# FitSNAP/FitSNAP

Hardware: AMD Instinct MI355X
Metric: training rows/sec through A^T A + solve, 1000000 x 128 fp64 in total over the GPUs (strong scaling) (higher is better)
Workload: dtype f64

## Files before the change

fitsnap_amd/csrc/fsnap_syrk.hip:

```cpp

#include <utility>

#include "fsnap_device_common.h"
#include "fsnap_kernels.h"

namespace {

__host__ __device__ constexpr int tri_index(int p, int q, int NB) {
    return p * NB - (p * (p - 1)) / 2 + (q - p);
}

__host__ __device__ inline int col_of(int bq, int e, int NB) {
    if ((NB & 1) && bq == NB - 1) return 16 * bq + e;
    return 32 * (bq >> 1) + 2 * e + (bq & 1);
}

__device__ __forceinline__ __amdgpu_buffer_rsrc_t make_rsrc(const void* p, unsigned bytes) {
    return __builtin_amdgcn_make_buffer_rsrc(const_cast<void*>(p), 0, (int)bytes, 0x00020000);
}

__device__ __forceinline__ double xlane_sum_rows(double x) {
    x += __shfl_xor(x, 16, 64);
    x += __shfl_xor(x, 32, 64);
    return x;
}

}

#ifdef FSNAP_TRACE
__device__ unsigned long long fsnap_trace_buf[4096 * 8];
__device__ unsigned long long fsnap_trace_wave[4096 * 16 * 4];
#define FSNAP_TRACE_CLK(v) const unsigned long long v = __builtin_readcyclecounter()
#endif

namespace {

template <int T, int NV>
__device__ __forceinline__ void acc_mfma(double a, double b, d4 (&vt)[NV]) {
    if constexpr (T < 32) {
        asm volatile("v_mfma_f64_16x16x4_f64 a[%2:%3], %0, %1, a[%2:%3]" : : "v"(a), "v"(b), "n"(8 * T), "n"(8 * T + 7));
    } else {
        asm volatile("v_mfma_f64_16x16x4_f64 %0, %1, %2, %0" : "+v"(vt[T - 32]) : "v"(a), "v"(b));
    }
}

template <int R>
__device__ __forceinline__ void acc_zero_reg() {
    asm volatile("v_accvgpr_write_b32 a[%0], 0" : : "n"(R));
}
template <int... R>
__device__ __forceinline__ void acc_zero_all(std::integer_sequence<int, R...>) {
    (acc_zero_reg<R>(), ...);
}

template <int T, int NV>
__device__ __forceinline__ d4 acc_read(const d4 (&vt)[NV]) {
    if constexpr (T >= 32) {
        return vt[T - 32];
    } else {
        unsigned r0, r1, r2, r3, r4, r5, r6, r7;
        asm volatile(
            "v_accvgpr_read_b32 %0, a[%8]\n\tv_accvgpr_read_b32 %1, a[%9]\n\t"
            "v_accvgpr_read_b32 %2, a[%10]\n\tv_accvgpr_read_b32 %3, a[%11]\n\t"
            "v_accvgpr_read_b32 %4, a[%12]\n\tv_accvgpr_read_b32 %5, a[%13]\n\t"
            "v_accvgpr_read_b32 %6, a[%14]\n\tv_accvgpr_read_b32 %7, a[%15]"
            : "=v"(r0), "=v"(r1), "=v"(r2), "=v"(r3), "=v"(r4), "=v"(r5), "=v"(r6), "=v"(r7)
            : "n"(8 * T), "n"(8 * T + 1), "n"(8 * T + 2), "n"(8 * T + 3), "n"(8 * T + 4), "n"(8 * T + 5), "n"(8 * T + 6),
              "n"(8 * T + 7));
        d4 x;
        x[0] = __builtin_bit_cast(double, ((unsigned long long)r1 << 32) | r0);
        x[1] = __builtin_bit_cast(double, ((unsigned long long)r3 << 32) | r2);
        x[2] = __builtin_bit_cast(double, ((unsigned long long)r5 << 32) | r4);
        x[3] = __builtin_bit_cast(double, ((unsigned long long)r7 << 32) | r6);
        return x;
    }
}

template <int TB, int N, int NV, int... U>
__device__ __forceinline__ void acc_read_range(d4 (&tmp)[N], const d4 (&vt)[NV], std::integer_sequence<int, U...>) {
    ((tmp[U] = acc_read<TB + U, NV>(vt)), ...);
}

template <int NB, int P, int NV, int... Q>
__device__ __forceinline__ void acc_row(const double (&V)[NB], d4 (&vt)[NV], std::integer_sequence<int, Q...>) {
    (acc_mfma<tri_index(P, P + Q, NB), NV>(V[P], V[P + Q], vt), ...);
}

template <int NB>
struct RawM {
    u4 pr[NB / 2 > 0 ? NB / 2 : 1];
    u2 tail;
    u4 wp;
};

constexpr unsigned FSNAP_OOB_VOFF = 0xFFFFF000u;

struct WaveBufsP {
    __amdgpu_buffer_rsrc_t A, wp;
    unsigned voffA;
    unsigned voffT;
    unsigned voffP;
    unsigned chunk_bytes;
};

__device__ __forceinline__ u4 load_pack(const WaveBufsP& wb, unsigned cl) {
    return __builtin_amdgcn_raw_buffer_load_b128(wb.wp, wb.voffP, cl * 64u, 0);
}
__device__ __forceinline__ bool pack_keep(const u4& wp) {
    return ((wp[0] | (wp[1] & 0x7FFFFFFFu)) != 0u);
}

template <int NB, bool NT>
__device__ __forceinline__ void issue_rows(RawM<NB>& r, const WaveBufsP& wb, unsigned cl) {
    const unsigned soff = cl * wb.chunk_bytes;
    constexpr int AUX = NT ? 2 : 0;
    const bool keep = pack_keep(r.wp);
    const unsigned va = keep ? wb.voffA : FSNAP_OOB_VOFF;
#pragma unroll
    for (int j = 0; j < NB / 2; ++j) r.pr[j] = __builtin_amdgcn_raw_buffer_load_b128(wb.A, va + 256u * j, soff, AUX);
    if (NB & 1) {
        const unsigned vtl = keep ? wb.voffT : FSNAP_OOB_VOFF;
        r.tail = __builtin_amdgcn_raw_buffer_load_b64(wb.A, vtl, soff, AUX);
    }
}

template <int NB, bool NT>
__device__ __forceinline__ void issue_rows_w(RawM<NB>& r, const u4& wp, const WaveBufsP& wb, unsigned cl) {
    const unsigned soff = cl * wb.chunk_bytes;
    constexpr int AUX = NT ? 2 : 0;
    const bool keep = pack_keep(wp);
    const unsigned va = keep ? wb.voffA : FSNAP_OOB_VOFF;
#pragma unroll
    for (int j = 0; j < NB / 2; ++j) r.pr[j] = __builtin_amdgcn_raw_buffer_load_b128(wb.A, va + 256u * j, soff, AUX);
    if (NB & 1) {
        const unsigned vtl = keep ? wb.voffT : FSNAP_OOB_VOFF;
        r.tail = __builtin_amdgcn_raw_buffer_load_b64(wb.A, vtl, soff, AUX);
    }
}

template <class F, int... I>
__device__ __forceinline__ void wave_p_for_impl(F&& f, std::integer_sequence<int, I...>) {
    (f(std::integral_constant<int, I>{}), ...);
}
template <int N, class F>
__device__ __forceinline__ void wave_p_for(F&& f) {
    wave_p_for_impl(f, std::make_integer_sequence<int, N>{});
}

template <int NB, bool NT, int P>
__device__ __forceinline__ void issue_piece(RawM<NB>& r, const WaveBufsP& wb, unsigned cl, unsigned va, unsigned vtl) {
    constexpr int AUX = NT ? 2 : 0;
    constexpr int NPR = NB / 2;
    const unsigned soff = cl * wb.chunk_bytes;
    if (P < NPR) r.pr[P] = __builtin_amdgcn_raw_buffer_load_b128(wb.A, va + 256u * P, soff, AUX);
    if ((NB & 1) && P == NPR) r.tail = __builtin_amdgcn_raw_buffer_load_b64(wb.A, vtl, soff, AUX);
    static_assert(NPR + (NB & 1) <= NB, "one load piece per MFMA slot");
}

template <int NB, bool FULLK>
__device__ __forceinline__ double weighted_block(const RawM<NB>& r, int j, double wv, int K, int e) {
    if ((NB & 1) && j == NB - 1) {
        const double x = wv * __builtin_bit_cast(double, r.tail);
        if (FULLK) return x;
        return (16 * (NB - 1) + e < K) ? x : 0.0;
    }
    const double x = wv * __builtin_bit_cast(d2, r.pr[j >> 1])[j & 1];
    constexpr int last_pair = (NB & 1) ? -1 : NB / 2 - 1;
    if (FULLK || (j >> 1) != last_pair) return x;
    return (32 * (j >> 1) + 2 * e + (j & 1) < K) ? x : 0.0;
}

template <bool PACK>
__device__ __forceinline__ u4 load_pack_x(const WaveBufsP& wb, const double* lpk, unsigned cl) {
    if constexpr (PACK) return __builtin_bit_cast(u4, *reinterpret_cast<const d2*>(lpk + (size_t)cl * 8));
    else return load_pack(wb, cl);
}

__device__ __forceinline__ void pack_rows_to_lds(const double* __restrict__ b, const double* __restrict__ w,
                                                 const unsigned char* __restrict__ mask, int64_t row0, int64_t nrow,
                                                 unsigned wave_rows, unsigned region_rows, double* lpw, int lane, double* sout) {
    constexpr int PB = 16;
    const __amdgpu_buffer_rsrc_t rb = make_rsrc(b + row0, (unsigned)(nrow * 8));
    const __amdgpu_buffer_rsrc_t rw_ = make_rsrc(w + row0, (unsigned)(nrow * 8));
    const __amdgpu_buffer_rsrc_t rm = make_rsrc(mask + row0, (unsigned)nrow);
    double bb = 0.0, sb = 0.0, cnt = 0.0;
    for (unsigned r0 = 0; r0 < wave_rows; r0 += 64u * PB) {
        u2 bv[PB], wv[PB];
        unsigned char mk[PB];
#pragma unroll
        for (int u = 0; u < PB; ++u) {
            const unsigned row = r0 + 64u * u + (unsigned)lane;
            bv[u] = __builtin_amdgcn_raw_buffer_load_b64(rb, row * 8u, 0, 0);
            wv[u] = __builtin_amdgcn_raw_buffer_load_b64(rw_, row * 8u, 0, 0);
            mk[u] = __builtin_amdgcn_raw_buffer_load_b8(rm, row, 0, 0);
        }
#pragma unroll
        for (int u = 0; u < PB; ++u) {
            const unsigned row = r0 + 64u * u + (unsigned)lane;
            const bool keep = (mk[u] != 0);
            const double wvv = keep ? __builtin_bit_cast(double, wv[u]) : 0.0;
            const double wbv = keep ? wvv * __builtin_bit_cast(double, bv[u]) : 0.0;
            if (row < wave_rows) {
                d2 o;
                o[0] = wvv;
                o[1] = wbv;
                *reinterpret_cast<d2*>(lpw + (size_t)row * 2) = o;
            }
            bb = __builtin_fma(wbv, wbv, bb);
            sb += wbv;
            cnt += keep ? 1.0 : 0.0;
        }
    }
    for (unsigned row = wave_rows + (unsigned)lane; row < region_rows; row += 64u) {
        const d2 z = {0.0, 0.0};
        *reinterpret_cast<d2*>(lpw + (size_t)row * 2) = z;
    }
#pragma unroll
    for (int sh = 1; sh < 64; sh <<= 1) {
        bb += __shfl_xor(bb, sh, 64);
        sb += __shfl_xor(sb, sh, 64);
        cnt += __shfl_xor(cnt, sh, 64);
    }
    if (lane == 0) {
        sout[0] = bb;
        sout[1] = sb;
        sout[2] = cnt;
        sout[3] = 0.0;
    }
}

template <int NB, bool FULLK, bool NT, int P>
__device__ __forceinline__ void acc_slot(double (&V)[NB], const RawM<NB>& RN, double wv, double wbv, double& wbp, int K,
                                         int e, double (&cacc)[NB], RawM<NB>& RF, const WaveBufsP& wb, unsigned cl_fill,
                                         unsigned va, unsigned vtl) {
#if !defined(FSNAP_ACC_ABL) || !(FSNAP_ACC_ABL & 1)
    issue_piece<NB, NT, P>(RF, wb, cl_fill, va, vtl);
#endif
    if (P == 0) cacc[NB - 1] = __builtin_fma(V[NB - 1], wbp, cacc[NB - 1]);
    else cacc[P - 1] = __builtin_fma(V[P - 1], wbv, cacc[P - 1]);
    V[P] = weighted_block<NB, FULLK>(RN, P, wv, K, e);
    if (P == NB - 1) wbp = wbv;
    __builtin_amdgcn_sched_barrier(0);
}

template <int NB, bool FULLK, bool NT, bool PACK, int NV, int... P>
__device__ __forceinline__ void acc_step(double (&V)[NB], d4 (&vt)[NV], RawM<NB>& RF, const RawM<NB>& RN, const WaveBufsP& wb,
                                         const double* lpk, unsigned cl_fill, int K, int e, double (&cacc)[NB], double& wbp,
                                         const u4& PW, const u4& PKEEP, u4& PLOAD, std::integer_sequence<int, P...>) {
    const d2 wpn = __builtin_bit_cast(d2, PW);
    const double wv = wpn[0], wbv = wpn[1];
    const bool keep = pack_keep(PKEEP);
    const unsigned va = keep ? wb.voffA : FSNAP_OOB_VOFF;
    const unsigned vtl = (NB & 1) ? (keep ? wb.voffT : FSNAP_OOB_VOFF) : 0u;
#if !defined(FSNAP_ACC_ABL) || !(FSNAP_ACC_ABL & 1)
    PLOAD = load_pack_x<PACK>(wb, lpk, cl_fill + 2);
#endif
    __builtin_amdgcn_sched_barrier(0);
#if defined(FSNAP_ACC_ABL) && (FSNAP_ACC_ABL & 2)
    (acc_row<NB, P>(V, vt, std::make_integer_sequence<int, NB - P>{}), ...);
    (void)wbv;
#else
    ((acc_row<NB, P>(V, vt, std::make_integer_sequence<int, NB - P>{}),
      acc_slot<NB, FULLK, NT, P>(V, RN, wv, wbv, wbp, K, e, cacc, RF, wb, cl_fill, va, vtl)),
     ...);
#endif
}

constexpr int FSNAP_ACC_LDS_DOUBLES = 20480;
constexpr int FSNAP_ACC_PACK_PAD = 12;

}

template <int NB, bool FULLK, bool NT, bool PACK>
__global__ __launch_bounds__(256) __attribute__((amdgpu_waves_per_eu(1, 1))) void
fsnap_syrk_acc(const double* __restrict__ A, int64_t lda, const double* __restrict__ wpack, int64_t m, int K,
               int64_t chunks_per_wave, double* __restrict__ part, double* __restrict__ cpart,
               const double* __restrict__ bvec, const double* __restrict__ wvec, const unsigned char* __restrict__ mask,
               double* __restrict__ spart) {

    constexpr int NTILE = NB * (NB + 1) / 2;
    constexpr int NV = NTILE > 32 ? NTILE - 32 : 1;
    constexpr int NPART = (NTILE * 1024 + FSNAP_ACC_LDS_DOUBLES - 1) / FSNAP_ACC_LDS_DOUBLES;
    constexpr int PER = (NTILE + NPART - 1) / NPART;
    static_assert(4 * PER * 256 <= FSNAP_ACC_LDS_DOUBLES, "fold part does not fit the LDS");
    __shared__ __attribute__((aligned(16))) double lds[FSNAP_ACC_LDS_DOUBLES];
#ifdef FSNAP_TRACE
    const unsigned long long trace_t0 = wall_clock64();
    const unsigned long long trace_c0 = __builtin_readcyclecounter();
#endif
    const int lane = threadIdx.x & 63, e = lane & 15, kr = lane >> 4;
    const int rw = __builtin_amdgcn_readfirstlane((int)(threadIdx.x >> 6));
    const int64_t rowwave = (int64_t)blockIdx.x * 4 + rw;
    const int64_t nchunks = (m + 3) >> 2;
    int64_t c0 = rowwave * chunks_per_wave;
    int64_t c1 = c0 + chunks_per_wave;
    if (c1 > nchunks) c1 = nchunks;
    if (c0 > c1) c0 = c1;
    const int64_t row0 = c0 << 2;
    int64_t row1 = c1 << 2;
    if (row1 > m) row1 = m;
    const int64_t nrow = row1 > row0 ? row1 - row0 : 0;
    WaveBufsP wb;
    wb.A = make_rsrc(A + row0 * lda, (unsigned)(nrow * lda * 8 + (nrow ? 16 : 0)));
    wb.wp = make_rsrc(PACK ? nullptr : wpack + 2 * row0, PACK ? 0u : (unsigned)(nrow * 16));
    wb.voffA = (unsigned)((kr * lda + 2 * e) * 8);
    wb.voffT = (unsigned)((kr * lda + 16 * (NB - 1) + e) * 8);
    wb.voffP = (unsigned)(kr * 16);
    wb.chunk_bytes = (unsigned)(lda * 32);
    const unsigned ncl = (unsigned)(c1 - c0);

    const double* lpk = nullptr;
    if constexpr (PACK) {
        const unsigned wave_rows = (unsigned)chunks_per_wave * 4u;
        const unsigned region_rows = wave_rows + FSNAP_ACC_PACK_PAD * 4u;
        double* lpw = lds + (size_t)rw * region_rows * 2;
        pack_rows_to_lds(bvec, wvec, mask, row0, nrow, wave_rows, region_rows, lpw, lane, spart + rowwave * 4);
        lpk = lpw + 2 * kr;
    }

    asm volatile("" : : : "a0", "a255");
    acc_zero_all(std::make_integer_sequence<int, 256>{});
    d4 vt[NV];
#pragma unroll
    for (int u = 0; u < NV; ++u) vt[u] = d4{0.0, 0.0, 0.0, 0.0};
    double cacc[NB], V[NB];
#pragma unroll
    for (int p = 0; p < NB; ++p) cacc[p] = 0.0;
    RawM<NB> r0, r1, r2;
    constexpr auto rows = std::make_integer_sequence<int, NB>{};
    if (ncl > 0) {
        r0.wp = load_pack_x<PACK>(wb, lpk, 0);
        r1.wp = load_pack_x<PACK>(wb, lpk, 1);
        r2.wp = load_pack_x<PACK>(wb, lpk, 2);
        issue_rows<NB, NT>(r0, wb, 0);
        issue_rows<NB, NT>(r1, wb, 1);
        issue_rows<NB, NT>(r2, wb, 2);
        {
            const d2 wp0 = __builtin_bit_cast(d2, r0.wp);
            const double wv = wp0[0], wbv = wp0[1];
#pragma unroll
            for (int p = 0; p < NB; ++p) {
                V[p] = weighted_block<NB, FULLK>(r0, p, wv, K, e);
                cacc[p] = __builtin_fma(V[p], wbv, cacc[p]);
            }
        }
        u4 pk0 = r0.wp, pk1 = r1.wp, pk2 = r2.wp, pk3 = load_pack_x<PACK>(wb, lpk, 3), pk4 = load_pack_x<PACK>(wb, lpk, 4),
           pk5 = {0u, 0u, 0u, 0u};
        (void)pk0;
        double wbp = 0.0;
        unsigned cl = 0;
        for (; cl + 3 < ncl; cl += 6) {
            acc_step<NB, FULLK, NT, PACK>(V, vt, r0, r1, wb, lpk, cl + 3, K, e, cacc, wbp, pk1, pk3, pk5, rows);
            acc_step<NB, FULLK, NT, PACK>(V, vt, r1, r2, wb, lpk, cl + 4, K, e, cacc, wbp, pk2, pk4, pk0, rows);
            acc_step<NB, FULLK, NT, PACK>(V, vt, r2, r0, wb, lpk, cl + 5, K, e, cacc, wbp, pk3, pk5, pk1, rows);
            acc_step<NB, FULLK, NT, PACK>(V, vt, r0, r1, wb, lpk, cl + 6, K, e, cacc, wbp, pk4, pk0, pk2, rows);
            acc_step<NB, FULLK, NT, PACK>(V, vt, r1, r2, wb, lpk, cl + 7, K, e, cacc, wbp, pk5, pk1, pk3, rows);
            acc_step<NB, FULLK, NT, PACK>(V, vt, r2, r0, wb, lpk, cl + 8, K, e, cacc, wbp, pk0, pk2, pk4, rows);
        }
        if (cl < ncl) {
            acc_step<NB, FULLK, NT, PACK>(V, vt, r0, r1, wb, lpk, cl + 3, K, e, cacc, wbp, pk1, pk3, pk5, rows);
            acc_step<NB, FULLK, NT, PACK>(V, vt, r1, r2, wb, lpk, cl + 4, K, e, cacc, wbp, pk2, pk4, pk0, rows);
            acc_step<NB, FULLK, NT, PACK>(V, vt, r2, r0, wb, lpk, cl + 5, K, e, cacc, wbp, pk3, pk5, pk1, rows);
        }
        cacc[NB - 1] = __builtin_fma(V[NB - 1], wbp, cacc[NB - 1]);
    }
    asm volatile("s_nop 15\n\ts_nop 15\n\ts_nop 15" : "+v"(vt[0]));
#pragma unroll
    for (int u = 1; u < NV; ++u) asm volatile("" : "+v"(vt[u]));
#ifdef FSNAP_TRACE
    if (threadIdx.x == 0 && blockIdx.x < 4096) {
        const int64_t wg = blockIdx.x;
        fsnap_trace_buf[wg * 8 + 0] = trace_t0;
        fsnap_trace_buf[wg * 8 + 1] = wall_clock64();
        fsnap_trace_buf[wg * 8 + 2] = __builtin_amdgcn_s_getreg((31 << 11) | 4);
        fsnap_trace_buf[wg * 8 + 3] = __builtin_amdgcn_s_getreg((3 << 11) | 20);
        fsnap_trace_buf[wg * 8 + 4] = __builtin_readcyclecounter() - trace_c0;
    }
#endif

    if constexpr (PACK) __syncthreads();
    double* pw = part + (int64_t)blockIdx.x * (int64_t)(NTILE * 256);
    auto fold_part = [&](auto part_tag) {
        constexpr int H = decltype(part_tag)::value;
        constexpr int TB = H * PER;
        constexpr int NT_H = (TB + PER <= NTILE) ? PER : (NTILE - TB);
        constexpr int Q = (NT_H + 3) / 4;
        double* slot = lds + (size_t)rw * PER * 256;
        {
            d4 tmp[NT_H];
            acc_read_range<TB>(tmp, vt, std::make_integer_sequence<int, NT_H>{});
#pragma unroll
            for (int u = 0; u < NT_H; ++u)
#pragma unroll
                for (int i = 0; i < 4; ++i) slot[(u * 4 + i) * 64 + lane] = tmp[u][i];
        }
        __syncthreads();
        for (int u = rw * Q; u < (rw + 1) * Q && u < NT_H; ++u) {
#pragma unroll
            for (int i = 0; i < 4; ++i) {
                const int o = (u * 4 + i) * 64 + lane;
                const double s01 = lds[o] + lds[PER * 256 + o];
                pw[((TB + u) * 4 + i) * 64 + lane] = (s01 + lds[2 * PER * 256 + o]) + lds[3 * PER * 256 + o];
            }
        }
        if (H + 1 < NPART) __syncthreads();
    };
    wave_p_for<NPART>(fold_part);

    double* cw = cpart + rowwave * (int64_t)(NB * 16);
#pragma unroll
    for (int p = 0; p < NB; ++p) {
        double sm = xlane_sum_rows(cacc[p]);
        if (kr == 0) cw[p * 16 + e] = sm;
    }
#ifdef FSNAP_TRACE
    if (threadIdx.x == 0 && blockIdx.x < 4096) fsnap_trace_buf[blockIdx.x * 8 + 5] = wall_clock64();
#endif
}

constexpr int FSNAP_WAVE_P_PACK_PAD = 16;

template <int NB, bool FULLK, bool NT, bool PACK>
__global__ __launch_bounds__(256, 2) void fsnap_syrk_wave_p(const double* __restrict__ A, int64_t lda,
                                                            const double* __restrict__ wpack, int64_t m, int K,
                                                            int64_t chunks_per_wave,
                                                            double* __restrict__ part, double* __restrict__ cpart,
                                                            const double* __restrict__ bvec, const double* __restrict__ wvec,
                                                            const unsigned char* __restrict__ mask,
                                                            double* __restrict__ spart) {
    constexpr int NTILE = NB * (NB + 1) / 2;
    extern __shared__ __attribute__((aligned(16))) double lds[];
    const int lane = threadIdx.x & 63, e = lane & 15, kr = lane >> 4;
    const int rw = __builtin_amdgcn_readfirstlane((int)(threadIdx.x >> 6));
    const int64_t rowwave = (int64_t)blockIdx.x * 4 + rw;
    const int64_t nchunks = (m + 3) >> 2;
    int64_t c0 = rowwave * chunks_per_wave, ncl64;
    const int64_t stride = 1;
    {
        int64_t c1 = c0 + chunks_per_wave;
        if (c1 > nchunks) c1 = nchunks;
        if (c0 > c1) c0 = c1;
        ncl64 = c1 - c0;
    }
    const int64_t row0 = c0 << 2;
    int64_t row1 = (c0 + ncl64) << 2;
    if (row1 > m) row1 = m;
    const int64_t nrow = (ncl64 > 0 && row1 > row0) ? row1 - row0 : 0;
    WaveBufsP wb;
    wb.A = make_rsrc(A + row0 * lda, (unsigned)(nrow * lda * 8 + (nrow ? 16 : 0)));
    wb.wp = make_rsrc(PACK ? nullptr : wpack + 2 * row0, PACK ? 0u : (unsigned)(nrow * 16));
    wb.voffA = (unsigned)((kr * lda + 2 * e) * 8);
    wb.voffT = (unsigned)((kr * lda + 16 * (NB - 1) + e) * 8);
    wb.voffP = (unsigned)(kr * 16);
    wb.chunk_bytes = (unsigned)(stride * lda * 32);
    const unsigned pack_bytes = (unsigned)(stride * 64);
    const unsigned ncl = (unsigned)ncl64;
    const double* lpk = nullptr;
    if constexpr (PACK) {
        const unsigned wave_rows = (unsigned)chunks_per_wave * 4u;
        const unsigned region_rows = wave_rows + FSNAP_WAVE_P_PACK_PAD * 4u;
        double* lpw = lds + (size_t)rw * region_rows * 2;
        pack_rows_to_lds(bvec, wvec, mask, row0, nrow, wave_rows, region_rows, lpw, lane, spart + rowwave * 4);
        lpk = lpw + 2 * kr;
    }
    auto load_pack_s = [&](unsigned cl) -> u4 {
        if constexpr (PACK) return __builtin_bit_cast(u4, *reinterpret_cast<const d2*>(lpk + (size_t)cl * 8));
        else return __builtin_amdgcn_raw_buffer_load_b128(wb.wp, wb.voffP, cl * pack_bytes, 0);
    };

    d4 acc[NTILE];
#pragma unroll
    for (int t = 0; t < NTILE; ++t) acc[t] = d4{0.0, 0.0, 0.0, 0.0};
    double cacc[NB], V[NB];
#pragma unroll
    for (int p = 0; p < NB; ++p) {
        cacc[p] = 0.0;
        V[p] = 0.0;
    }
    double wbcur = 0.0;
    constexpr int D = NB <= 2 ? 4 : 3, W = 2 * D;
    RawM<NB> R[D];
    u4 P[W];
    if (ncl > 0) {
        wave_p_for<W - 1>([&](auto x) { P[x] = load_pack_s((unsigned)x); });
        wave_p_for<D>([&](auto x) { issue_rows_w<NB, NT>(R[x], P[x], wb, (unsigned)x); });
        {
            const d2 wp0 = __builtin_bit_cast(d2, P[0]);
#pragma unroll
            for (int p = 0; p < NB; ++p) V[p] = weighted_block<NB, FULLK>(R[0], p, wp0[0], K, e);
            wbcur = wp0[1];
        }
        for (unsigned cl = 0; cl < ncl; cl += W) {
            wave_p_for<W>([&](auto u_) {
                constexpr int u = decltype(u_)::value;
                const d2 wpn = __builtin_bit_cast(d2, P[(u + 1) % W]);
                P[(u + W - 1) % W] = load_pack_s(cl + u + W - 1);
                issue_rows_w<NB, NT>(R[u % D], P[(u + D) % W], wb, cl + u + D);
                __builtin_amdgcn_sched_barrier(0);
#pragma unroll
                for (int p = 0; p < NB; ++p) {
#pragma unroll
                    for (int q = p; q < NB; ++q) {
                        acc[tri_index(p, q, NB)] =
                            __builtin_amdgcn_mfma_f64_16x16x4f64(V[p], V[q], acc[tri_index(p, q, NB)], 0, 0, 0);
                    }
                }
#pragma unroll
                for (int p = 0; p < NB; ++p) cacc[p] = __builtin_fma(V[p], wbcur, cacc[p]);
#pragma unroll
                for (int p = 0; p < NB; ++p) V[p] = weighted_block<NB, FULLK>(R[(u + 1) % D], p, wpn[0], K, e);
                wbcur = wpn[1];
                __builtin_amdgcn_sched_barrier(0);
            });
        }
    }

    if constexpr (PACK) __syncthreads();
    {
        double* slot_hi = lds + (size_t)((rw & 1) * NTILE) * 256;
        if (rw >= 2) {
#pragma unroll
            for (int u = 0; u < NTILE; ++u)
#pragma unroll
                for (int i = 0; i < 4; ++i) slot_hi[(u * 4 + i) * 64 + lane] = acc[u][i];
        }
        __syncthreads();
        if (rw < 2) {
#pragma unroll
            for (int u = 0; u < NTILE; ++u)
#pragma unroll
                for (int i = 0; i < 4; ++i) acc[u][i] += slot_hi[(u * 4 + i) * 64 + lane];
        }
        __syncthreads();
        if (rw == 1) {
#pragma unroll
            for (int u = 0; u < NTILE; ++u)
#pragma unroll
                for (int i = 0; i < 4; ++i) lds[(u * 4 + i) * 64 + lane] = acc[u][i];
        }
        __syncthreads();
        if (rw == 0) {
            double* pw = part + (int64_t)blockIdx.x * (int64_t)(NTILE * 256);
#pragma unroll
            for (int u = 0; u < NTILE; ++u)
#pragma unroll
                for (int i = 0; i < 4; ++i) pw[(u * 4 + i) * 64 + lane] = acc[u][i] + lds[(u * 4 + i) * 64 + lane];
        }
    }
    double* cw = cpart + rowwave * (int64_t)(NB * 16);
#pragma unroll
    for (int p = 0; p < NB; ++p) {
        double sm = xlane_sum_rows(cacc[p]);
        if (kr == 0) cw[p * 16 + e] = sm;
    }
}

__global__ __launch_bounds__(256) void fsnap_reduce_partials2(const double* __restrict__ part,
                                                              const double* __restrict__ cpart,
                                                              const double* __restrict__ spart, int nblocks,
                                                              int cs_per_block, int ns, int NB, int K,
                                                              double* __restrict__ out, double* __restrict__ mirror,
                                                              int accumulate, int upper_mirror) {
    __shared__ __attribute__((aligned(16))) double red[16][32];
    const int NTILE = NB * (NB + 1) / 2;
    const int nG = NTILE * 256, nC = NB * 16;
    const int gG = nG / 32, gC = (nC + 31) / 32;
    const int tid = threadIdx.x, sub = tid & 15, slice = tid >> 4;
    const int b = blockIdx.x;
    int region, e0, nel, np;
    const double* src;
    int64_t stride;
    if (b < gG) {
        region = 0; e0 = b * 32; nel = nG; np = nblocks; src = part; stride = nG;
    } else if (b < gG + gC) {
        region = 1; e0 = (b - gG) * 32; nel = nC; np = nblocks * cs_per_block; src = cpart; stride = nC;
    } else {
        region = 2; e0 = 0; nel = 4; np = ns >= 0 ? ns : nblocks * cs_per_block; src = spart; stride = 4;
    }
    const int el = e0 + 2 * sub;
    d2 a0 = {0.0, 0.0}, a1 = a0, a2 = a0, a3 = a0;
    if (el < nel) {
        const double* s0 = src + el;
        int p = slice;
        for (; p + 240 < np; p += 256) {
            d2 x[16];
#pragma unroll
            for (int j = 0; j < 16; ++j) x[j] = *reinterpret_cast<const d2*>(s0 + (int64_t)(p + 16 * j) * stride);
#pragma unroll
            for (int j = 0; j < 16; j += 4) {
                a0 += x[j];
                a1 += x[j + 1];
                a2 += x[j + 2];
                a3 += x[j + 3];
            }
        }
        for (; p < np; p += 16) a0 += *reinterpret_cast<const d2*>(s0 + (int64_t)p * stride);
    }
    const d2 sv = (a0 + a1) + (a2 + a3);
    *reinterpret_cast<d2*>(&red[slice][2 * sub]) = sv;
    __syncthreads();
    if (tid >= 32) return;
    const int idx = e0 + tid;
    if (idx >= nel) return;
    double tot = red[0][tid];
#pragma unroll
    for (int k = 1; k < 16; ++k) tot += red[k][tid];
    if (region == 0) {
        const int t = idx >> 8, rem = idx & 255, i = rem >> 6, ln = rem & 63;
        int p = 0;
        while (p + 1 < NB && tri_index(p + 1, p + 1, NB) <= t) ++p;
        const int q = p + (t - tri_index(p, p, NB));
        const int ep = (ln >> 4) + 4 * i, eq = ln & 15;
        const int r = col_of(p, ep, NB), c = col_of(q, eq, NB);
        if (r < K && c < K) {
            const double val = accumulate ? out[(int64_t)r * K + c] + tot : tot;
            out[(int64_t)r * K + c] = val;
            if (p != q) out[(int64_t)c * K + r] = val;
            if (mirror) {
                if (upper_mirror) {
                    const int lo = r < c ? r : c, hi = r < c ? c : r;
                    if (p != q) mirror[(int64_t)lo * K + hi] = val;
                    else mirror[(int64_t)r * K + c] = val;
                } else {
                    mirror[(int64_t)r * K + c] = val;
                    if (p != q) mirror[(int64_t)c * K + r] = val;
                }
                if (r == c) mirror[(int64_t)K * K + K + 3 + r] = val;
            }
        }
    } else if (region == 1) {
        const int cidx = col_of(idx >> 4, idx & 15, NB);
        if (cidx < K) {
            const double val = accumulate ? out[(int64_t)K * K + cidx] + tot : tot;
            out[(int64_t)K * K + cidx] = val;
            if (mirror) mirror[(int64_t)K * K + cidx] = val;
        }
    } else if (idx < 3) {
        const double val = accumulate ? out[(int64_t)K * K + K + idx] + tot : tot;
        out[(int64_t)K * K + K + idx] = val;
        if (mirror) mirror[(int64_t)K * K + K + idx] = val;
    }
}

namespace {

struct RawT {
    u4 pi[2], pj[2];
    u4 wp;
};

struct WaveBufsT {
    __amdgpu_buffer_rsrc_t A, wp;
    unsigned voffP;
    unsigned chunk_bytes;
};

__device__ __forceinline__ u4 load_pack_t(const WaveBufsT& wb, unsigned cl) {
    return __builtin_amdgcn_raw_buffer_load_b128(wb.wp, wb.voffP, cl * 64u, 0);
}
__device__ __forceinline__ u2 load_pack_w(const WaveBufsT& wb, unsigned cl) {
    return __builtin_amdgcn_raw_buffer_load_b64(wb.wp, wb.voffP, cl * 64u, 0);
}
__device__ __forceinline__ bool pack_keep_w(const u2& wp) { return ((wp[0] | (wp[1] & 0x7FFFFFFFu)) != 0u); }
template <bool DIAG>
__device__ __forceinline__ void load_pack_d(u4& dst, const WaveBufsT& wb, unsigned cl) {
    if (DIAG) {
        dst = load_pack_t(wb, cl);
    } else {
        const u2 t = load_pack_w(wb, cl);
        dst[0] = t[0];
        dst[1] = t[1];
    }
}

template <bool DIAG, int EDGE, bool NT>
__device__ __forceinline__ void issue_rows_t(RawT& r, const WaveBufsT& wb, unsigned voffI, unsigned voffJ, unsigned cl) {
    const unsigned soff = cl * wb.chunk_bytes;
    constexpr int AUX = NT ? 2 : 0;
    const bool keep = pack_keep(r.wp);
    const unsigned vi = keep ? voffI : FSNAP_OOB_VOFF;
    r.pi[0] = __builtin_amdgcn_raw_buffer_load_b128(wb.A, vi, soff, AUX);
    if (!(DIAG && EDGE == 2)) r.pi[1] = __builtin_amdgcn_raw_buffer_load_b128(wb.A, vi + 256u, soff, AUX);
    if (!DIAG) {
        const unsigned vj = keep ? voffJ : FSNAP_OOB_VOFF;
        r.pj[0] = __builtin_amdgcn_raw_buffer_load_b128(wb.A, vj, soff, AUX);
        if (EDGE != 2) r.pj[1] = __builtin_amdgcn_raw_buffer_load_b128(wb.A, vj + 256u, soff, AUX);
    }
}

template <bool DIAG, int EDGE, bool NT>
__device__ __forceinline__ void issue_rows_tw(RawT& r, const u4& wp, const WaveBufsT& wb, unsigned voffI, unsigned voffJ,
                                              unsigned cl) {
    const unsigned soff = cl * wb.chunk_bytes;
    constexpr int AUX = NT ? 2 : 0;
    const bool keep = pack_keep(wp);
    const unsigned vi = keep ? voffI : FSNAP_OOB_VOFF;
    r.pi[0] = __builtin_amdgcn_raw_buffer_load_b128(wb.A, vi, soff, AUX);
    if (!(DIAG && EDGE == 2)) r.pi[1] = __builtin_amdgcn_raw_buffer_load_b128(wb.A, vi + 256u, soff, AUX);
    if (!DIAG) {
        const unsigned vj = keep ? voffJ : FSNAP_OOB_VOFF;
        r.pj[0] = __builtin_amdgcn_raw_buffer_load_b128(wb.A, vj, soff, AUX);
        if (EDGE != 2) r.pj[1] = __builtin_amdgcn_raw_buffer_load_b128(wb.A, vj + 256u, soff, AUX);
    }
}

template <bool DIAG, int EDGE>
__device__ __forceinline__ void prep_t(double (&vI)[4], double (&vJ)[4], const RawT& r, double wv, int colI0, int colJ0,
                                       int K, int e) {
    const double f = DIAG ? wv : wv * wv;
#pragma unroll
    for (int j = 0; j < 2; ++j) {
        if (!(DIAG && EDGE == 2 && j == 1)) {
            const d2 x = __builtin_bit_cast(d2, r.pi[j]);
            vI[2 * j] = f * x[0];
            vI[2 * j + 1] = f * x[1];
            if (DIAG && EDGE) {
                if (!(colI0 + 32 * j + 2 * e < K)) vI[2 * j] = 0.0;
                if (!(colI0 + 32 * j + 2 * e + 1 < K)) vI[2 * j + 1] = 0.0;
            }
        }
        if (!DIAG && !(EDGE == 2 && j == 1)) {
            const d2 y = __builtin_bit_cast(d2, r.pj[j]);
            vJ[2 * j] = y[0];
            vJ[2 * j + 1] = y[1];
            if (EDGE) {
                if (!(colJ0 + 32 * j + 2 * e < K)) vJ[2 * j] = 0.0;
                if (!(colJ0 + 32 * j + 2 * e + 1 < K)) vJ[2 * j + 1] = 0.0;
            }
        }
    }
}

template <bool DIAG, int EDGE, bool NT, bool RING = false>
__device__ __forceinline__ void syrk_tiled_body(const double* __restrict__ A, int64_t lda,
                                                const double* __restrict__ wpack, int64_t m, int K, int I, int J,
                                                int64_t c0, int64_t c1, int wv_in_wg, double* lds,
                                                double* __restrict__ pw, double* __restrict__ cw) {
    constexpr int NTW = 16;
    const int lane = threadIdx.x & 63, e = lane & 15, kr = lane >> 4;
    d4 acc[NTW];
#pragma unroll
    for (int t = 0; t < NTW; ++t) acc[t] = d4{0.0, 0.0, 0.0, 0.0};
    double cacc[4] = {0.0, 0.0, 0.0, 0.0};

    const int64_t row0 = c0 << 2;
    int64_t row1 = c1 << 2;
    if (row1 > m) row1 = m;
    const int64_t nrow = row1 > row0 ? row1 - row0 : 0;
    WaveBufsT wb;
    wb.A = make_rsrc(A + row0 * lda, (unsigned)(nrow * lda * 8 + (nrow ? 16 : 0)));
    wb.wp = make_rsrc(wpack + 2 * row0, (unsigned)(nrow * 16));
    wb.voffP = (unsigned)(kr * 16);
    wb.chunk_bytes = (unsigned)(lda * 32);
    const unsigned voffI = (unsigned)((kr * lda + 64 * I + 2 * e) * 8);
    const unsigned voffJ = (unsigned)((kr * lda + 64 * J + 2 * e) * 8);
    const unsigned ncl = (unsigned)(c1 > c0 ? c1 - c0 : 0);

    RawT r0, r1, r2;
    double vI[4] = {0.0, 0.0, 0.0, 0.0}, vJ[4] = {0.0, 0.0, 0.0, 0.0};
    double wbcur = 0.0;
    constexpr int QMAX = (EDGE == 2) ? 2 : 4;
    constexpr int PMAX = (DIAG && EDGE == 2) ? 2 : 4;

    if constexpr (RING) {
        constexpr int D = 3, W = 6;
        RawT R[D];
        u4 P[W];
        if (ncl > 0) {
            wave_p_for<W - 1>([&](auto x) { load_pack_d<DIAG>(P[x], wb, (unsigned)x); });
            wave_p_for<D>([&](auto x) { issue_rows_tw<DIAG, EDGE, NT>(R[x], P[x], wb, voffI, voffJ, (unsigned)x); });
            {
                const d2 wp0 = __builtin_bit_cast(d2, P[0]);
                prep_t<DIAG, EDGE>(vI, vJ, R[0], wp0[0], 64 * I, 64 * J, K, e);
                wbcur = wp0[1];
            }
            for (unsigned cl = 0; cl < ncl; cl += W) {
                wave_p_for<W>([&](auto u_) {
                    constexpr int u = decltype(u_)::value;
                    const d2 wpn = __builtin_bit_cast(d2, P[(u + 1) % W]);
                    load_pack_d<DIAG>(P[(u + W - 1) % W], wb, cl + u + W - 1);
                    issue_rows_tw<DIAG, EDGE, NT>(R[u % D], P[(u + D) % W], wb, voffI, voffJ, cl + u + D);
                    __builtin_amdgcn_sched_barrier(0);
#pragma unroll
                    for (int p = 0; p < PMAX; ++p) {
#pragma unroll
                        for (int q = (DIAG ? p : 0); q < QMAX; ++q)
                            acc[p * 4 + q] = __builtin_amdgcn_mfma_f64_16x16x4f64(vI[p], DIAG ? vI[q] : vJ[q], acc[p * 4 + q], 0, 0, 0);
                    }
                    if (DIAG) {
#pragma unroll
                        for (int p = 0; p < PMAX; ++p) cacc[p] = __builtin_fma(vI[p], wbcur, cacc[p]);
                    }
                    prep_t<DIAG, EDGE>(vI, vJ, R[(u + 1) % D], wpn[0], 64 * I, 64 * J, K, e);
                    wbcur = wpn[1];
                    __builtin_amdgcn_sched_barrier(0);
                });
            }
        }
    } else {
#define FSNAP_STEP_T(RF, RN, CLF)                                                               \
    {                                                                                           \
        const d2 wpn = __builtin_bit_cast(d2, RN.wp);                                           \
        load_pack_d<DIAG>(RN.wp, wb, (CLF) + 1);                                                \
        issue_rows_t<DIAG, EDGE, NT>(RF, wb, voffI, voffJ, (CLF));                                    \
        _Pragma("unroll") for (int p = 0; p < PMAX; ++p) {                                      \
            _Pragma("unroll") for (int q = (DIAG ? p : 0); q < QMAX; ++q) {                     \
                acc[p * 4 + q] = __builtin_amdgcn_mfma_f64_16x16x4f64(vI[p], DIAG ? vI[q] : vJ[q], acc[p * 4 + q], 0, 0, 0); \
            }                                                                                   \
        }                                                                                       \
        if (DIAG) {                                                                             \
            _Pragma("unroll") for (int p = 0; p < PMAX; ++p) cacc[p] = __builtin_fma(vI[p], wbcur, cacc[p]); \
        }                                                                                       \
        prep_t<DIAG, EDGE>(vI, vJ, RN, wpn[0], 64 * I, 64 * J, K, e);                           \
        wbcur = wpn[1];                                                                         \
    }
    if (ncl > 0) {
        load_pack_d<DIAG>(r0.wp, wb, 0);
        load_pack_d<DIAG>(r1.wp, wb, 1);
        load_pack_d<DIAG>(r2.wp, wb, 2);
        issue_rows_t<DIAG, EDGE, NT>(r0, wb, voffI, voffJ, 0);
        issue_rows_t<DIAG, EDGE, NT>(r1, wb, voffI, voffJ, 1);
        issue_rows_t<DIAG, EDGE, NT>(r2, wb, voffI, voffJ, 2);
        {
            const d2 wp0 = __builtin_bit_cast(d2, r0.wp);
            prep_t<DIAG, EDGE>(vI, vJ, r0, wp0[0], 64 * I, 64 * J, K, e);
            wbcur = wp0[1];
        }
        load_pack_d<DIAG>(r0.wp, wb, 3);
        for (unsigned cl = 0; cl < ncl; cl += 3) {
            FSNAP_STEP_T(r0, r1, cl + 3)
            FSNAP_STEP_T(r1, r2, cl + 4)
            FSNAP_STEP_T(r2, r0, cl + 5)
        }
    }
#undef FSNAP_STEP_T
    }

    {
        const int rw = wv_in_wg;
        double* slot_hi = lds + (size_t)((rw & 1) * NTW) * 256;
        if (rw >= 2) {
#pragma unroll
            for (int u = 0; u < NTW; ++u)
#pragma unroll
                for (int i = 0; i < 4; ++i) slot_hi[(u * 4 + i) * 64 + lane] = acc[u][i];
        }
        __syncthreads();
        if (rw < 2) {
#pragma unroll
            for (int u = 0; u < NTW; ++u)
#pragma unroll
                for (int i = 0; i < 4; ++i) acc[u][i] += slot_hi[(u * 4 + i) * 64 + lane];
        }
        __syncthreads();
        if (rw == 1) {
#pragma unroll
            for (int u = 0; u < NTW; ++u)
#pragma unroll
                for (int i = 0; i < 4; ++i) lds[(u * 4 + i) * 64 + lane] = acc[u][i];
        }
        __syncthreads();
        if (rw == 0) {
#pragma unroll
            for (int u = 0; u < NTW; ++u)
#pragma unroll
                for (int i = 0; i < 4; ++i) pw[(u * 4 + i) * 64 + lane] = acc[u][i] + lds[(u * 4 + i) * 64 + lane];
        }
    }
    if (DIAG) {
#pragma unroll
        for (int p = 0; p < 4; ++p) {
            double s = xlane_sum_rows(cacc[p]);
            if (kr == 0) cw[p * 16 + e] = s;
        }
    }
}

}

template <bool NT>
__global__ __launch_bounds__(256, 2) void fsnap_syrk_tiled(const double* __restrict__ A, int64_t lda,
                                                           const double* __restrict__ wpack, int64_t m, int K,
                                                           int NSB, int npairs, int64_t chunks_per_split,
                                                           int nitems,
                                                           double* __restrict__ part, double* __restrict__ cpart) {
    __shared__ double lds[2 * 16 * 256];
    const int wv = __builtin_amdgcn_readfirstlane((int)(threadIdx.x >> 6));
    unsigned item = blockIdx.x;
    int I, J, split;
    {
        const unsigned per = ((unsigned)nitems + 7u) >> 3;
        const unsigned slot = blockIdx.x >> 3;
        item = (blockIdx.x & 7u) * per + slot;
        if (slot >= per || item >= (unsigned)nitems) return;
    }
    const int id = (int)(item % (unsigned)npairs);
    split = (int)(item / (unsigned)npairs);
    const int noff = npairs - NSB;
    if (id < noff) {
        I = 0;
        int rem = id;
        while (rem >= NSB - 1 - I) {
            rem -= NSB - 1 - I;
            ++I;
        }
        J = I + 1 + rem;
    } else {
        I = J = id - noff;
    }
    const int pair = I * NSB - (I * (I - 1)) / 2 + (J - I);
    const int64_t nchunks = (m + 3) >> 2;
    const int64_t cpw = (chunks_per_split + 3) >> 2;
    int64_t s0 = (int64_t)split * chunks_per_split;
    int64_t s1 = s0 + chunks_per_split;
    if (s1 > nchunks) s1 = nchunks;
    int64_t c0 = s0 + (int64_t)wv * cpw;
    int64_t c1 = c0 + cpw;
    if (c1 > s1) c1 = s1;
    if (c0 > s1) c0 = s1;
    double* pw = part + ((int64_t)split * npairs + pair) * (16 * 256);
    double* cw = cpart + (((int64_t)split * NSB + I) * 4 + wv) * 64;
    const int tail = K & 63;
    const int edge = (J == NSB - 1 && tail != 0) ? (tail <= 32 ? 2 : 4) : 0;
    if (I == J) {
        if (edge == 2) syrk_tiled_body<true, 2, NT, true>(A, lda, wpack, m, K, I, J, c0, c1, wv, lds, pw, cw);
        else if (edge == 4) syrk_tiled_body<true, 4, NT, true>(A, lda, wpack, m, K, I, J, c0, c1, wv, lds, pw, cw);
        else syrk_tiled_body<true, 0, NT, true>(A, lda, wpack, m, K, I, J, c0, c1, wv, lds, pw, cw);
    } else {
        if (edge == 2) syrk_tiled_body<false, 2, NT, true>(A, lda, wpack, m, K, I, J, c0, c1, wv, lds, pw, cw);
        else if (edge == 4) syrk_tiled_body<false, 4, NT, true>(A, lda, wpack, m, K, I, J, c0, c1, wv, lds, pw, cw);
        else syrk_tiled_body<false, 0, NT, true>(A, lda, wpack, m, K, I, J, c0, c1, wv, lds, pw, cw);
    }
}

__device__ __forceinline__ void reduce_tiled_store_g(int64_t idx, double tot, int NSB, int K, double* __restrict__ out,
                                                     int accumulate) {
    const int pair = (int)(idx >> 12), rem = (int)(idx & 4095);
    const int t = rem >> 8, i = (rem >> 6) & 3, ln = rem & 63;
    int I = 0, pr = pair;
    while (pr >= NSB - I) {
        pr -= NSB - I;
        ++I;
    }
    const int J = I + pr;
    const int p = t >> 2, q = t & 3;
    if (I == J && q < p) return;
    const int ep = (ln >> 4) + 4 * i, eq = ln & 15;
    const int r = 64 * I + 32 * (p >> 1) + 2 * ep + (p & 1);
    const int c = 64 * J + 32 * (q >> 1) + 2 * eq + (q & 1);
    if (r < K && c < K) {
        const double val = accumulate ? out[(int64_t)r * K + c] + tot : tot;
        out[(int64_t)r * K + c] = val;
        if (!(I == J && p == q)) out[(int64_t)c * K + r] = val;
    }
}


__global__ __launch_bounds__(256) void fsnap_reduce_tiled_small(const double* __restrict__ part, int nsplit, int NSB,
                                                                int npairs, int K, double* __restrict__ out,
                                                                int accumulate) {
    const int64_t nG = (int64_t)npairs * 4096;
    const int64_t idx = (int64_t)blockIdx.x * 256 + threadIdx.x;
    if (idx >= nG) return;
    double tot = 0.0;
    for (int p = 0; p < nsplit; ++p) tot += part[(int64_t)p * nG + idx];
    reduce_tiled_store_g(idx, tot, NSB, K, out, accumulate);
}

__global__ __launch_bounds__(1024) void fsnap_reduce_tiled(const double* __restrict__ part,
                                                           const double* __restrict__ cpart,
                                                           const double* __restrict__ spart, int ns, int nsplit, int NSB,
                                                           int npairs, int K, double* __restrict__ out, int accumulate,
                                                           int64_t idx0) {
    __shared__ double red[1024];
    const int64_t nG = (int64_t)npairs * 4096;
    const int nC = NSB * 64, nS = 4;
    const int tid = threadIdx.x, g = tid >> 6, l = tid & 63;
    const int64_t idx = idx0 + (int64_t)blockIdx.x * 64 + l;
    const double* src = nullptr;
    int64_t stride = 0;
    int np = 0;
    if (idx < nG) {
        src = part + idx;
        stride = nG;
        np = nsplit;
    } else if (idx < nG + nC) {
        const int j = (int)(idx - nG);
        src = cpart + (int64_t)(j >> 6) * 256 + (j & 63);
        stride = 0;
        np = nsplit * 4;
    } else if (idx < nG + nC + nS) {
        src = spart + (idx - nG - nC);
        stride = 4;
        np = ns;
    }
    double s = 0.0;
    if (src) {
        if (idx >= nG && idx < nG + nC) {
            for (int q = g; q < np; q += 16) {
                const int split = q >> 2, wave = q & 3;
                s += src[((int64_t)split * NSB * 4 + wave) * 64];
            }
        } else {
            int p = g;
            double a0 = 0.0, a1 = 0.0, a2 = 0.0, a3 = 0.0;
            for (; p + 48 < np; p += 64) {
                const double x0 = src[(int64_t)p * stride], x1 = src[(int64_t)(p + 16) * stride];
                const double x2 = src[(int64_t)(p + 32) * stride], x3 = src[(int64_t)(p + 48) * stride];
                a0 += x0; a1 += x1; a2 += x2; a3 += x3;
            }
            for (; p < np; p += 16) a0 += src[(int64_t)p * stride];
            s = (a0 + a1) + (a2 + a3);
        }
    }
    red[tid] = s;
    __syncthreads();
    if (g == 0 && src) {
        double tot = 0.0;
#pragma unroll
        for (int k = 0; k < 16; ++k) tot += red[k * 64 + l];
        if (idx < nG) {
            reduce_tiled_store_g(idx, tot, NSB, K, out, accumulate);
        } else if (idx < nG + nC) {
            const int j = (int)(idx - nG);
            const int Ib = j >> 6, bq = (j >> 4) & 3, e = j & 15;
            const int cidx = 64 * Ib + 32 * (bq >> 1) + 2 * e + (bq & 1);
            if (cidx < K) out[(int64_t)K * K + cidx] = accumulate ? out[(int64_t)K * K + cidx] + tot : tot;
        } else {
            const int j = (int)(idx - nG - nC);
            if (j < 3) out[(int64_t)K * K + K + j] = accumulate ? out[(int64_t)K * K + K + j] + tot : tot;
        }
    }
}

namespace fsnap {

int syrk_num_blocks(int K) { return (K + 15) / 16; }

int syrk_waves_per_simd(int K, int split) {
    const int NB = syrk_num_blocks(K);
    const int ntw = (NB * (NB + 1) / 2 + split - 1) / split;
    const int regs = 8 * ntw + 12 * NB + 40;
    int wps = 512 / regs;
    if (wps < 1) wps = 1;
    if (wps > 8) wps = 8;
    return wps;
}

template <int NB>
static hipError_t launch_syrk_acc_nb(const SyrkArgs& a, hipStream_t st) {
    dim3 grid((unsigned)a.nblocks), block(256);
    const bool fullk = (a.K == 16 * NB);
    if (a.fused_pack ? (!a.b || !a.w || !a.mask || !a.spart) : !a.wpack) return hipErrorInvalidValue;
#define FSNAP_LAUNCH(FK, NTL, PK)                                                                                   \
    hipLaunchKernelGGL((fsnap_syrk_acc<NB, FK, NTL, PK>), grid, block, 0, st, a.A, a.lda, a.wpack, a.m, a.K,        \
                       a.chunks_per_wave, a.part, a.cpart, a.b, a.w, a.mask, a.spart)
#define FSNAP_LAUNCH_PK(FK, NTL)                 \
    do {                                         \
        if (a.fused_pack) FSNAP_LAUNCH(FK, NTL, true); \
        else FSNAP_LAUNCH(FK, NTL, false);       \
    } while (0)
    if (fullk) {
        if (a.nontemporal) FSNAP_LAUNCH_PK(true, true);
        else FSNAP_LAUNCH_PK(true, false);
    } else {
        if (a.nontemporal) FSNAP_LAUNCH_PK(false, true);
        else FSNAP_LAUNCH_PK(false, false);
    }
#undef FSNAP_LAUNCH_PK
#undef FSNAP_LAUNCH
    return hipGetLastError();
}

template <int NB>
static hipError_t launch_syrk_wave_p_nb(const SyrkArgs& a, hipStream_t st) {
    dim3 grid((unsigned)a.nblocks), block(256);
    const bool fullk = (a.K == 16 * NB);
    if (a.fused_pack ? (!a.b || !a.w || !a.mask || !a.spart) : !a.wpack) return hipErrorInvalidValue;
    constexpr size_t fold_bytes = (size_t)2 * (NB * (NB + 1) / 2) * 256 * sizeof(double);
    const size_t pair_bytes = a.fused_pack ? (size_t)4 * (size_t)(a.chunks_per_wave + FSNAP_WAVE_P_PACK_PAD) * 64 : 0;
    const size_t lds = pair_bytes > fold_bytes ? pair_bytes : fold_bytes;
    if (lds > 64 * 1024) return hipErrorInvalidValue;
#define FSNAP_LAUNCH(FK, NTL, PK)                                                                                      \
    hipLaunchKernelGGL((fsnap_syrk_wave_p<NB, FK, NTL, PK>), grid, block, lds, st, a.A, a.lda, a.wpack, a.m, a.K,       \
                       a.chunks_per_wave, a.part, a.cpart, a.b, a.w, a.mask, a.spart)
#define FSNAP_LAUNCH_PK(FK, NTL)                       \
    do {                                               \
        if (a.fused_pack) FSNAP_LAUNCH(FK, NTL, true); \
        else FSNAP_LAUNCH(FK, NTL, false);             \
    } while (0)
    if (fullk) {
        if (a.nontemporal) FSNAP_LAUNCH_PK(true, true);
        else FSNAP_LAUNCH_PK(true, false);
    } else {
        if (a.nontemporal) FSNAP_LAUNCH_PK(false, true);
        else FSNAP_LAUNCH_PK(false, false);
    }
#undef FSNAP_LAUNCH_PK
#undef FSNAP_LAUNCH
    return hipGetLastError();
}

int64_t syrk_wave_p_max_fused_cpw(int K, int wg_per_cu) {
    const int NB = syrk_num_blocks(K);
    const int64_t fold_bytes = (int64_t)2 * (NB * (NB + 1) / 2) * 256 * 8;
    int64_t budget = (int64_t)160 * 1024 / (wg_per_cu > 0 ? wg_per_cu : 1);
    if (budget > 64 * 1024) budget = 64 * 1024;
    if (budget < fold_bytes) budget = fold_bytes;
    return budget / 256 - FSNAP_WAVE_P_PACK_PAD;
}

hipError_t launch_syrk_wave_p(const SyrkArgs& a, hipStream_t st) {
    switch (syrk_num_blocks(a.K)) {
        case 1: return launch_syrk_wave_p_nb<1>(a, st);
        case 2: return launch_syrk_wave_p_nb<2>(a, st);
        case 3: return launch_syrk_wave_p_nb<3>(a, st);
        case 4: return launch_syrk_wave_p_nb<4>(a, st);
        case 5: return launch_syrk_wave_p_nb<5>(a, st);
        default: return hipErrorInvalidValue;
    }
}

int64_t syrk_acc_max_fused_cpw() { return FSNAP_ACC_LDS_DOUBLES / 32 - FSNAP_ACC_PACK_PAD; }

hipError_t launch_syrk_acc(const SyrkArgs& a, hipStream_t st) {
    switch (syrk_num_blocks(a.K)) {
        case 6: return launch_syrk_acc_nb<6>(a, st);
        case 7: return launch_syrk_acc_nb<7>(a, st);
        case 8: return launch_syrk_acc_nb<8>(a, st);
        case 9: return launch_syrk_acc_nb<9>(a, st);
        default: return hipErrorInvalidValue;
    }
}

hipError_t launch_reduce(const double* part, const double* cpart, const double* spart, int nblocks,
                         int cs_per_block, int ns, int K, double* out, double* mirror, bool accumulate, hipStream_t st,
                         bool upper_mirror) {
    const int NB = syrk_num_blocks(K);
    const int ngroups = NB * (NB + 1) / 2 * 8 + (NB * 16 + 31) / 32 + 1;
    hipLaunchKernelGGL(fsnap_reduce_partials2, dim3((unsigned)ngroups), dim3(256), 0, st, part, cpart, spart, nblocks,
                       cs_per_block, ns, NB, K, out, mirror, accumulate ? 1 : 0, upper_mirror ? 1 : 0);
    return hipGetLastError();
}

hipError_t launch_syrk_tiled(const TiledArgs& a, hipStream_t st) {
    const int nitems = (int)((int64_t)a.npairs * a.nsplit);
    const int64_t per_xcd = (nitems + 7) / 8;
    dim3 grid((unsigned)(8 * per_xcd)), block(256);
    if (a.nontemporal)
        hipLaunchKernelGGL((fsnap_syrk_tiled<true>), grid, block, 0, st, a.A, a.lda, a.wpack, a.m, a.K, a.NSB,
                           a.npairs, a.chunks_per_split, nitems, a.part, a.cpart);
    else
        hipLaunchKernelGGL((fsnap_syrk_tiled<false>), grid, block, 0, st, a.A, a.lda, a.wpack, a.m, a.K, a.NSB,
                           a.npairs, a.chunks_per_split, nitems, a.part, a.cpart);
    return hipGetLastError();
}

hipError_t launch_reduce_tiled(const TiledArgs& a, double* out, bool accumulate, hipStream_t st) {
    const int64_t nG = (int64_t)a.npairs * 4096, nrest = a.NSB * 64 + 4;
    if (a.nsplit <= 16) {
        hipLaunchKernelGGL(fsnap_reduce_tiled_small, dim3((unsigned)((nG + 255) / 256)), dim3(256), 0, st, a.part, a.nsplit, a.NSB,
                           a.npairs, a.K, out, accumulate ? 1 : 0);
        hipLaunchKernelGGL(fsnap_reduce_tiled, dim3((unsigned)((nrest + 63) / 64)), dim3(1024), 0, st, a.part, a.cpart, a.spart, a.ns,
                           a.nsplit, a.NSB, a.npairs, a.K, out, accumulate ? 1 : 0, nG);
        return hipGetLastError();
    }
    const int64_t nelem = nG + nrest;
    dim3 grid((unsigned)((nelem + 63) / 64)), block(1024);
    hipLaunchKernelGGL(fsnap_reduce_tiled, grid, block, 0, st, a.part, a.cpart, a.spart, a.ns, a.nsplit, a.NSB, a.npairs, a.K,
                       out, accumulate ? 1 : 0, (int64_t)0);
    return hipGetLastError();
}

}
```

Before: 3.154 billion.

## Issue first A-row loads during weight packing and gate rows afterwards

Moves the first three chunk loads of A (issued without the mask gate) and the accumulator zeroing into a hook that runs inside the LDS packing loop, right after the b/w/mask loads are issued. The rows are then zeroed by the mask once the pack values are available. This overlaps the A-load latency with the prologue packing work. The tail loop is also rewritten so it runs only the remaining 1-5 steps instead of always three or six. A trace timestamp is added under the trace build flag.

```diff
diff --git a/fitsnap_amd/csrc/fsnap_syrk.hip b/fitsnap_amd/csrc/fsnap_syrk.hip
--- a/fitsnap_amd/csrc/fsnap_syrk.hip
+++ b/fitsnap_amd/csrc/fsnap_syrk.hip
@@ -138,6 +138,27 @@
     }
 }
 
+template <int NB, bool NT>
+__device__ __forceinline__ void issue_rows_ungated(RawM<NB>& r, const WaveBufsP& wb, unsigned cl) {
+    const unsigned soff = cl * wb.chunk_bytes;
+    constexpr int AUX = NT ? 2 : 0;
+#pragma unroll
+    for (int j = 0; j < NB / 2; ++j) r.pr[j] = __builtin_amdgcn_raw_buffer_load_b128(wb.A, wb.voffA + 256u * j, soff, AUX);
+    if (NB & 1) r.tail = __builtin_amdgcn_raw_buffer_load_b64(wb.A, wb.voffT, soff, AUX);
+}
+template <int NB>
+__device__ __forceinline__ void gate_rows(RawM<NB>& r) {
+    const bool keep = pack_keep(r.wp);
+#pragma unroll
+    for (int j = 0; j < NB / 2; ++j)
+#pragma unroll
+        for (int i = 0; i < 4; ++i) r.pr[j][i] = keep ? r.pr[j][i] : 0u;
+    if (NB & 1) {
+        r.tail[0] = keep ? r.tail[0] : 0u;
+        r.tail[1] = keep ? r.tail[1] : 0u;
+    }
+}
+
 template <class F, int... I>
 __device__ __forceinline__ void wave_p_for_impl(F&& f, std::integer_sequence<int, I...>) {
     (f(std::integral_constant<int, I>{}), ...);
@@ -176,9 +197,14 @@
     else return load_pack(wb, cl);
 }
 
+struct PackNoHook {
+    __device__ __forceinline__ void operator()() const {}
+};
+template <class Hook = PackNoHook>
 __device__ __forceinline__ void pack_rows_to_lds(const double* __restrict__ b, const double* __restrict__ w,
                                                  const unsigned char* __restrict__ mask, int64_t row0, int64_t nrow,
-                                                 unsigned wave_rows, unsigned region_rows, double* lpw, int lane, double* sout) {
+                                                 unsigned wave_rows, unsigned region_rows, double* lpw, int lane, double* sout,
+                                                 Hook&& hook = Hook{}) {
     constexpr int PB = 16;
     const __amdgpu_buffer_rsrc_t rb = make_rsrc(b + row0, (unsigned)(nrow * 8));
     const __amdgpu_buffer_rsrc_t rw_ = make_rsrc(w + row0, (unsigned)(nrow * 8));
@@ -194,6 +220,7 @@
             wv[u] = __builtin_amdgcn_raw_buffer_load_b64(rw_, row * 8u, 0, 0);
             mk[u] = __builtin_amdgcn_raw_buffer_load_b8(rm, row, 0, 0);
         }
+        if (r0 == 0) hook();
 #pragma unroll
         for (int u = 0; u < PB; ++u) {
             const unsigned row = r0 + 64u * u + (unsigned)lane;
@@ -287,6 +314,7 @@
 #ifdef FSNAP_TRACE
     const unsigned long long trace_t0 = wall_clock64();
     const unsigned long long trace_c0 = __builtin_readcyclecounter();
+    unsigned long long trace_t1 = trace_t0;
 #endif
     const int lane = threadIdx.x & 63, e = lane & 15, kr = lane >> 4;
     const int rw = __builtin_amdgcn_readfirstlane((int)(threadIdx.x >> 6));
@@ -309,32 +337,43 @@
     wb.chunk_bytes = (unsigned)(lda * 32);
     const unsigned ncl = (unsigned)(c1 - c0);
 
+    RawM<NB> r0, r1, r2;
+    auto start_rows = [&]() {
+        issue_rows_ungated<NB, NT>(r0, wb, 0);
+        issue_rows_ungated<NB, NT>(r1, wb, 1);
+        issue_rows_ungated<NB, NT>(r2, wb, 2);
+        __builtin_amdgcn_sched_barrier(0);
+        asm volatile("" : : : "a0", "a255");
+        acc_zero_all(std::make_integer_sequence<int, 256>{});
+        __builtin_amdgcn_sched_barrier(0);
+    };
     const double* lpk = nullptr;
     if constexpr (PACK) {
         const unsigned wave_rows = (unsigned)chunks_per_wave * 4u;
         const unsigned region_rows = wave_rows + FSNAP_ACC_PACK_PAD * 4u;
         double* lpw = lds + (size_t)rw * region_rows * 2;
-        pack_rows_to_lds(bvec, wvec, mask, row0, nrow, wave_rows, region_rows, lpw, lane, spart + rowwave * 4);
+        pack_rows_to_lds(bvec, wvec, mask, row0, nrow, wave_rows, region_rows, lpw, lane, spart + rowwave * 4, start_rows);
         lpk = lpw + 2 * kr;
-    }
-
-    asm volatile("" : : : "a0", "a255");
-    acc_zero_all(std::make_integer_sequence<int, 256>{});
-    d4 vt[NV];
-#pragma unroll
-    for (int u = 0; u < NV; ++u) vt[u] = d4{0.0, 0.0, 0.0, 0.0};
-    double cacc[NB], V[NB];
-#pragma unroll
-    for (int p = 0; p < NB; ++p) cacc[p] = 0.0;
-    RawM<NB> r0, r1, r2;
-    constexpr auto rows = std::make_integer_sequence<int, NB>{};
-    if (ncl > 0) {
         r0.wp = load_pack_x<PACK>(wb, lpk, 0);
         r1.wp = load_pack_x<PACK>(wb, lpk, 1);
         r2.wp = load_pack_x<PACK>(wb, lpk, 2);
-        issue_rows<NB, NT>(r0, wb, 0);
-        issue_rows<NB, NT>(r1, wb, 1);
-        issue_rows<NB, NT>(r2, wb, 2);
+    } else {
+        r0.wp = load_pack_x<PACK>(wb, lpk, 0);
+        r1.wp = load_pack_x<PACK>(wb, lpk, 1);
+        r2.wp = load_pack_x<PACK>(wb, lpk, 2);
+        start_rows();
+    }
+    d4 vt[NV];
+#pragma unroll
+    for (int u = 0; u < NV; ++u) vt[u] = d4{0.0, 0.0, 0.0, 0.0};
+    double cacc[NB], V[NB];
+#pragma unroll
+    for (int p = 0; p < NB; ++p) cacc[p] = 0.0;
+    constexpr auto rows = std::make_integer_sequence<int, NB>{};
+    if (ncl > 0) {
+        gate_rows<NB>(r0);
+        gate_rows<NB>(r1);
+        gate_rows<NB>(r2);
         {
             const d2 wp0 = __builtin_bit_cast(d2, r0.wp);
             const double wv = wp0[0], wbv = wp0[1];
@@ -348,20 +387,36 @@
            pk5 = {0u, 0u, 0u, 0u};
         (void)pk0;
         double wbp = 0.0;
+#define FSNAP_ACC_STEP(RF, RN, D, PW, PKEEP, PLOAD) \
+    acc_step<NB, FULLK, NT, PACK>(V, vt, RF, RN, wb, lpk, cl + D, K, e, cacc, wbp, PW, PKEEP, PLOAD, rows)
+#ifdef FSNAP_TRACE
+        trace_t1 = wall_clock64();
+#endif
+        const unsigned ncl6 = ncl - ncl % 6u;
         unsigned cl = 0;
-        for (; cl + 3 < ncl; cl += 6) {
-            acc_step<NB, FULLK, NT, PACK>(V, vt, r0, r1, wb, lpk, cl + 3, K, e, cacc, wbp, pk1, pk3, pk5, rows);
-            acc_step<NB, FULLK, NT, PACK>(V, vt, r1, r2, wb, lpk, cl + 4, K, e, cacc, wbp, pk2, pk4, pk0, rows);
-            acc_step<NB, FULLK, NT, PACK>(V, vt, r2, r0, wb, lpk, cl + 5, K, e, cacc, wbp, pk3, pk5, pk1, rows);
-            acc_step<NB, FULLK, NT, PACK>(V, vt, r0, r1, wb, lpk, cl + 6, K, e, cacc, wbp, pk4, pk0, pk2, rows);
-            acc_step<NB, FULLK, NT, PACK>(V, vt, r1, r2, wb, lpk, cl + 7, K, e, cacc, wbp, pk5, pk1, pk3, rows);
-            acc_step<NB, FULLK, NT, PACK>(V, vt, r2, r0, wb, lpk, cl + 8, K, e, cacc, wbp, pk0, pk2, pk4, rows);
-        }
-        if (cl < ncl) {
-            acc_step<NB, FULLK, NT, PACK>(V, vt, r0, r1, wb, lpk, cl + 3, K, e, cacc, wbp, pk1, pk3, pk5, rows);
-            acc_step<NB, FULLK, NT, PACK>(V, vt, r1, r2, wb, lpk, cl + 4, K, e, cacc, wbp, pk2, pk4, pk0, rows);
-            acc_step<NB, FULLK, NT, PACK>(V, vt, r2, r0, wb, lpk, cl + 5, K, e, cacc, wbp, pk3, pk5, pk1, rows);
-        }
+        for (; cl < ncl6; cl += 6) {
+            FSNAP_ACC_STEP(r0, r1, 3, pk1, pk3, pk5);
+            FSNAP_ACC_STEP(r1, r2, 4, pk2, pk4, pk0);
+            FSNAP_ACC_STEP(r2, r0, 5, pk3, pk5, pk1);
+            FSNAP_ACC_STEP(r0, r1, 6, pk4, pk0, pk2);
+            FSNAP_ACC_STEP(r1, r2, 7, pk5, pk1, pk3);
+            FSNAP_ACC_STEP(r2, r0, 8, pk0, pk2, pk4);
+        }
+        const unsigned left = ncl - cl;
+        if (left > 0) {
+            FSNAP_ACC_STEP(r0, r1, 3, pk1, pk3, pk5);
+            if (left > 1) {
+                FSNAP_ACC_STEP(r1, r2, 4, pk2, pk4, pk0);
+                if (left > 2) {
+                    FSNAP_ACC_STEP(r2, r0, 5, pk3, pk5, pk1);
+                    if (left > 3) {
+                        FSNAP_ACC_STEP(r0, r1, 6, pk4, pk0, pk2);
+                        if (left > 4) FSNAP_ACC_STEP(r1, r2, 7, pk5, pk1, pk3);
+                    }
+                }
+            }
+        }
+#undef FSNAP_ACC_STEP
         cacc[NB - 1] = __builtin_fma(V[NB - 1], wbp, cacc[NB - 1]);
     }
     asm volatile("s_nop 15\n\ts_nop 15\n\ts_nop 15" : "+v"(vt[0]));
@@ -375,6 +430,7 @@
         fsnap_trace_buf[wg * 8 + 2] = __builtin_amdgcn_s_getreg((31 << 11) | 4);
         fsnap_trace_buf[wg * 8 + 3] = __builtin_amdgcn_s_getreg((3 << 11) | 20);
         fsnap_trace_buf[wg * 8 + 4] = __builtin_readcyclecounter() - trace_c0;
+        fsnap_trace_buf[wg * 8 + 6] = trace_t1;
     }
 #endif
 
```

Result: slower. 3.103 billion (-1.6%).
